# snakers4/silero-vad

Measured on AMD Instinct MI355X. Metric: audio-chunks/sec (32 ms @ 16 kHz), higher is better.
Workload: dtype f32; 1 GPU; configs[1]: synthetic 16 kHz PCM resident in HBM, 512-sample chunks, 4096 streams/GPU x 256 chunks/stream per step, zero initial state; streams_per_gpu=4096

## Files before the change

### silero_vad_amd/csrc/fft_wave.hpp

```cpp
#pragma once
#include <hip/hip_runtime.h>

#include "device_api.hpp"
#include "layout.hpp"

#ifndef VAD_NT_PCM
#define VAD_NT_PCM 0
#endif

namespace vad {
namespace {

using f32x4 = float __attribute__((ext_vector_type(4)));
using u32x4 = unsigned __attribute__((ext_vector_type(4)));

#ifndef VAD_TRACE
#define VAD_TRACE 0
#endif
#ifndef VAD_ABLATE
#define VAD_ABLATE 0
#endif

__device__ constexpr float kCos32[16] = {1.0f, 0.98078525f, 0.9238795f, 0.8314696f, 0.70710677f,
    0.55557024f, 0.38268343f, 0.19509032f, 0.0f, -0.19509032f, -0.38268343f, -0.55557024f,
    -0.70710677f, -0.8314696f, -0.9238795f, -0.98078525f};
__device__ constexpr float kSin32[16] = {0.0f, 0.19509032f, 0.38268343f, 0.55557024f, 0.70710677f,
    0.8314696f, 0.9238795f, 0.98078525f, 1.0f, 0.98078525f, 0.9238795f, 0.8314696f, 0.70710677f,
    0.55557024f, 0.38268343f, 0.19509032f};

constexpr int bitrev(int x, int bits) {
    int r = 0;
    for (int i = 0; i < bits; ++i) r |= ((x >> i) & 1) << (bits - 1 - i);
    return r;
}
constexpr int ilog2(int x) { return x <= 1 ? 0 : 1 + ilog2(x / 2); }

struct Lane {
    int lane, g, j, wave;
    long t;
    long tl;
    long st;
    int b;
    bool tile_valid;
    bool from_tail;
    float sgnA, sgnB;
#if VAD_TRACE
    mutable unsigned long long ts[20] = {};
#endif
};
#if VAD_TRACE
#define VAD_WAVE_STAMP(ln, slot) do { (ln).ts[(slot)] = __builtin_readcyclecounter(); } while (0)
#else
#define VAD_WAVE_STAMP(ln, slot) do { } while (0)
#endif

__device__ __forceinline__ void cvt8(const u32x4 v, float *o) {
#pragma unroll
    for (int k = 0; k < 4; ++k) {
        const int lo = (int)(v[k] << 16) >> 16, hi = (int)v[k] >> 16;
        o[2 * k] = (float)lo * (1.0f / 32768.0f);
        o[2 * k + 1] = (float)hi * (1.0f / 32768.0f);
    }
}
template <int SL, int DEC>
__device__ __forceinline__ void load_vec(const float *p, float (&s)[SL]) {
    if (DEC == 1) {
#pragma unroll
        for (int k = 0; k < SL / 4; ++k) {
            const f32x4 v = VAD_NT_PCM ? __builtin_nontemporal_load(reinterpret_cast<const f32x4 *>(p) + k)
                                       : reinterpret_cast<const f32x4 *>(p)[k];
#pragma unroll
            for (int e = 0; e < 4; ++e) s[4 * k + e] = v[e];
        }
    } else {
#pragma unroll
        for (int i = 0; i < SL; ++i) s[i] = p[i * DEC];
        __builtin_amdgcn_sched_barrier(0);
    }
}
template <int SL, int DEC>
__device__ __forceinline__ void load_vec(const int16_t *p, float (&s)[SL]) {
    if (DEC == 1) {
#pragma unroll
        for (int k = 0; k < SL / 8; ++k)
            cvt8(VAD_NT_PCM ? __builtin_nontemporal_load(reinterpret_cast<const u32x4 *>(p) + k)
                            : reinterpret_cast<const u32x4 *>(p)[k], &s[8 * k]);
    } else {
#pragma unroll
        for (int h = 0; h < 2; ++h) {
#pragma unroll
            for (int i = h * SL / 2; i < (h + 1) * SL / 2; ++i) s[i] = (float)p[i * DEC] * (1.0f / 32768.0f);
            __builtin_amdgcn_sched_barrier(0);
        }
    }
}

template <int Q, typename PcmT, int DEC>
__device__ __forceinline__ void load_slice(float (&s)[2 * Q], const FrontArgs &a, const Lane &ln, const int V) {
    constexpr int SL = 2 * Q, N = 16 * Q;
    const PcmT *row = reinterpret_cast<const PcmT *>(a.pcm) + (size_t)ln.b * a.ld;
    const int sigma = 2 * V + ln.g;
    const int sg = (V == 3 && sigma > 8) ? 8 : sigma;
    const long p0 = (long)SL * (8 * ln.t - 1 + sg);
    const PcmT *src = row + p0 * DEC;
    const PcmT *esrc = row + ((long)N * ln.t + N - SL - 1) * DEC;
    if (ln.from_tail) {
        const PcmT *trow = reinterpret_cast<const PcmT *>(a.tail) + (size_t)ln.b * N * DEC;
        if (sg > 0) src = trow + SL * (sg - 1) * DEC;
        esrc = trow + (N - SL - 1) * DEC;
    }
    if (VAD_ABLATE & 16) {
        const PcmT *r0 = reinterpret_cast<const PcmT *>(a.pcm) + (size_t)(ln.st * 16) * a.ld + (long)SL * 8 * ln.t;
#pragma unroll
        for (int k = 0; k < SL / 4; ++k) {
            const f32x4 v = *reinterpret_cast<const f32x4 *>(reinterpret_cast<const float *>(r0) + (size_t)(k & 15) * a.ld + ln.lane * 4);
#pragma unroll
            for (int e = 0; e < 4; ++e) s[4 * k + e] = v[e];
        }
    } else if (VAD_ABLATE & 32) {
        const float *rr = reinterpret_cast<const float *>(row) + (long)SL * 8 * ln.t;
#pragma unroll
        for (int k = 0; k < SL / 4; ++k) {
            const f32x4 v = *reinterpret_cast<const f32x4 *>(rr + 16 * k + 4 * ln.g + 128 * V);
#pragma unroll
            for (int e = 0; e < 4; ++e) s[4 * k + e] = v[e];
        }
    } else if (DEC == 1) {
        if (V == 0 && ln.t == 0 && ln.g == 0) load_vec<SL, 1>(a.ctx_in + (size_t)ln.b * SL, s);
        else load_vec<SL, 1>(src, s);
    } else if (V == 0) {
        const bool from_ctx = ln.t == 0 && ln.g == 0;
        const PcmT *safe = ln.from_tail ? reinterpret_cast<const PcmT *>(a.tail) + (size_t)ln.b * N * DEC : row;
        load_vec<SL, DEC>(from_ctx ? safe : src, s);
        const f32x4 *c4 = reinterpret_cast<const f32x4 *>(a.ctx_in + (size_t)ln.b * SL);
#pragma unroll
        for (int k = 0; k < SL / 4; ++k) {
            const f32x4 v = c4[k];
#pragma unroll
            for (int e = 0; e < 4; ++e) s[4 * k + e] = from_ctx ? v[e] : s[4 * k + e];
        }
    } else {
        load_vec<SL, DEC>(src, s);
    }
    if (V == 3) {
        if (a.ctx_out && ln.t == a.T - 1 && ln.g == 2 && ln.tile_valid &&
            (ln.st * 16 + ln.j) < a.B) {
            float *o = a.ctx_out + (size_t)ln.b * SL;
#pragma unroll
            for (int k = 0; k < SL / 4; ++k)
                reinterpret_cast<f32x4 *>(o)[k] = f32x4{s[4 * k], s[4 * k + 1], s[4 * k + 2], s[4 * k + 3]};
        }
        const bool rev = ln.g == 3;
        float extra = 0.f;
        if (rev) extra = load_pcm(esrc);
#pragma unroll
        for (int i = 0; i < SL / 2 - 1; ++i) {
            const int k = SL - 2 - i;
            const float lo = s[i], hi = s[k];
            s[i] = rev ? hi : lo;
            s[k] = rev ? lo : hi;
        }
        s[SL - 1] = rev ? extra : s[SL - 1];
    }
}

using f32x2 = float __attribute__((ext_vector_type(2)));

__device__ __forceinline__ f32x2 swap2(f32x2 v) { return f32x2{v.y, v.x}; }
__device__ __forceinline__ f32x2 cmul(f32x2 v, float c, float sn) {
    return __builtin_elementwise_fma(swap2(v), f32x2{-sn, sn}, v * f32x2{c, c});
}

#ifndef VAD_XLANE_SWAP
#define VAD_XLANE_SWAP 1
#endif
__device__ __forceinline__ void trade32(f32x2 &a, f32x2 &b) {
#pragma unroll
    for (int e = 0; e < 2; ++e) {
        const auto r = __builtin_amdgcn_permlane32_swap(__float_as_uint(a[e]), __float_as_uint(b[e]), false, false);
        a[e] = __uint_as_float(r[0]);
        b[e] = __uint_as_float(r[1]);
    }
}
__device__ __forceinline__ void trade16(f32x2 &a, f32x2 &b) {
#pragma unroll
    for (int e = 0; e < 2; ++e) {
        const auto r = __builtin_amdgcn_permlane16_swap(__float_as_uint(a[e]), __float_as_uint(b[e]), false, false);
        a[e] = __uint_as_float(r[0]);
        b[e] = __uint_as_float(r[1]);
    }
}

template <int Q>
__device__ __forceinline__ void fft_inlane(f32x2 (&z)[Q]) {
#pragma unroll
    for (int n = Q; n >= 2; n >>= 1) {
        const int half = n >> 1;
#pragma unroll
        for (int b0 = 0; b0 < Q; b0 += n) {
#pragma unroll
            for (int jx = 0; jx < half; ++jx) {
                const int i0 = b0 + jx, i1 = i0 + half;
                const f32x2 u = z[i0], v = z[i1];
                z[i0] = u + v;
                const f32x2 d = u - v;
                const int tw = jx * (32 / n);
                if (tw == 0) z[i1] = d;
                else if (tw == 8) z[i1] = swap2(d) * f32x2{1.0f, -1.0f};
                else z[i1] = cmul(d, kCos32[tw], -kSin32[tw]);
            }
        }
    }
}

template <int Q>
__device__ __forceinline__ void fft_math(float (&X)[Q + 1], const float (&s)[2 * Q], const float *tab_lds, const Lane &ln);

template <int Q, typename PcmT, int DEC = 1>
__device__ __forceinline__ void fft_frame(float (&X)[Q + 1], const int V, const FrontArgs &a, const float *tab_lds,
                                          const Lane &ln) {
    constexpr int SL = 2 * Q;
    __builtin_amdgcn_sched_barrier(0);
    VAD_WAVE_STAMP(ln, 16 + V);
    float s[SL];
    if (VAD_ABLATE & 4) {
#pragma unroll
        for (int i = 0; i < SL; ++i) s[i] = (float)(ln.lane + i) * 1e-3f;
    } else {
        load_slice<Q, PcmT, DEC>(s, a, ln, V);
    }
#if VAD_TRACE
    asm volatile("s_waitcnt vmcnt(0)" ::: "memory");
    VAD_WAVE_STAMP(ln, 2 + 2 * V);
#endif
    if (VAD_ABLATE & 2) {
#pragma unroll
        for (int k = 0; k < Q; ++k) X[k] = s[k] + s[k + Q];
        X[Q] = s[0];
        return;
    }
    fft_math<Q>(X, s, tab_lds, ln);
    VAD_WAVE_STAMP(ln, 3 + 2 * V);
}

template <int Q>
__device__ __forceinline__ void fft_math(float (&X)[Q + 1], const float (&s)[2 * Q], const float *tab_lds, const Lane &ln) {
    constexpr int SL = 2 * Q;
    constexpr vadl::Tab tb = vadl::make_tab(8 * Q, Q);

    f32x2 z[Q];
    {
        const f32x4 *w = reinterpret_cast<const f32x4 *>(tab_lds + tb.window + SL * ln.g);
#pragma unroll
        for (int k = 0; k < SL / 4; ++k) {
            const f32x4 wv = w[k];
            z[2 * k] = f32x2{s[4 * k], s[4 * k + 1]} * f32x2{wv[0], wv[1]};
            z[2 * k + 1] = f32x2{s[4 * k + 2], s[4 * k + 3]} * f32x2{wv[2], wv[3]};
        }
    }
    const f32x4 *tw1 = reinterpret_cast<const f32x4 *>(tab_lds + tb.tw1 + ln.g * Q * 4);
#if VAD_XLANE_SWAP
    constexpr int H = Q / 2;
    const f32x2 rotA = (ln.g & 1) ? f32x2{0.f, 0.f} : f32x2{1.f, 1.f};
    const f32x2 rotB = (ln.g & 1) ? f32x2{1.f, -1.f} : f32x2{0.f, 0.f};
#pragma unroll
    for (int q = 0; q < H; ++q) trade32(z[q], z[q + H]);
#pragma unroll
    for (int q = 0; q < H; ++q) {
        const f32x2 u = z[q], v = z[q + H], d = u - v;
        z[q] = u + v;
        z[q + H] = __builtin_elementwise_fma(swap2(d), rotB, d * rotA);
    }
#pragma unroll
    for (int q = 0; q < H; ++q) trade32(z[q], z[q + H]);
#pragma unroll
    for (int q = 0; q < H; ++q) trade16(z[q], z[q + H]);
#pragma unroll
    for (int q = 0; q < H; ++q) {
        const f32x2 u = z[q], v = z[q + H];
        z[q] = u + v;
        z[q + H] = u - v;
    }
#pragma unroll
    for (int q = 0; q < H; ++q) trade16(z[q], z[q + H]);
#pragma unroll
    for (int q = 0; q < Q; ++q) {
        const f32x2 x = z[q];
        const f32x4 t = tw1[q];
        z[q] = __builtin_elementwise_fma(swap2(x), f32x2{t[0], t[1]}, x * f32x2{t[2], t[2]});
    }
#else
    const f32x2 sA{ln.sgnA, ln.sgnA}, sB{ln.sgnB, ln.sgnB};
    const f32x2 rotA = ln.g == 3 ? f32x2{0.f, 0.f} : f32x2{1.f, 1.f};
    const f32x2 rotB = ln.g == 3 ? f32x2{1.f, -1.f} : f32x2{0.f, 0.f};
#pragma unroll
    for (int q = 0; q < Q; ++q) {
        f32x2 x = z[q];
        const f32x2 p{__shfl_xor(x.x, 32), __shfl_xor(x.y, 32)};
        x = __builtin_elementwise_fma(sA, x, p);
        x = __builtin_elementwise_fma(swap2(x), rotB, x * rotA);
        const f32x2 r{__shfl_xor(x.x, 16), __shfl_xor(x.y, 16)};
        x = __builtin_elementwise_fma(sB, x, r);
        const f32x4 t = tw1[q];
        z[q] = __builtin_elementwise_fma(swap2(x), f32x2{t[0], t[1]}, x * f32x2{t[2], t[2]});
    }
#endif
    fft_inlane<Q>(z);
    constexpr int LG = ilog2(Q);
    const f32x4 *tw2 = reinterpret_cast<const f32x4 *>(tab_lds + tb.tw2 + ln.g * Q * 4);
    const int src_lane4 = (ln.g >= 2 ? (ln.lane ^ 16) : ln.lane) * 4;
#pragma unroll
    for (int k = 0; k < Q; ++k) {
        const f32x2 u = z[bitrev(k, LG)];
        const int ks = bitrev((Q - k) % Q, LG), kr = bitrev(Q - 1 - k, LG);
        const f32x2 own = z[kr], alt = z[ks];
        const float xr = __int_as_float(__builtin_amdgcn_ds_bpermute(src_lane4, __float_as_int(own.x)));
        const float xi = __int_as_float(__builtin_amdgcn_ds_bpermute(src_lane4, __float_as_int(own.y)));
        const f32x2 p{ln.g == 0 ? alt.x : xr, ln.g == 0 ? alt.y : xi};
        const f32x2 av = __builtin_elementwise_fma(p, f32x2{1.0f, -1.0f}, u);
        const f32x2 ev = __builtin_elementwise_fma(p, f32x2{-1.0f, 1.0f}, u);
        const f32x4 t = tw2[k];
        const f32x2 y = __builtin_elementwise_fma(swap2(ev), f32x2{t[0], t[1]},
                                                  __builtin_elementwise_fma(ev, f32x2{t[2], t[2]}, av));
        const f32x2 yy = y * y;
        X[k] = 0.5f * __builtin_amdgcn_sqrtf(yy.x + yy.y);
    }
    X[Q] = ln.g == 0 ? fabsf(z[0].x - z[0].y) : 0.f;
}

template <int Q>
__device__ __forceinline__ void poison_acc(float &p0, float &p1, const float (&X)[Q + 1]) {
#pragma unroll
    for (int k = 0; k < Q; k += 2) {
        p0 = fmaf(X[k], 0.f, p0);
        p1 = fmaf(X[k + 1], 0.f, p1);
    }
}
__device__ __forceinline__ float poison_nyq(float p0, float p1, float xn0, float xn1, float xn2, float xn3) {
    p0 = fmaf(xn0, 0.f, p0);
    p1 = fmaf(xn1, 0.f, p1);
    p0 = fmaf(xn2, 0.f, p0);
    p1 = fmaf(xn3, 0.f, p1);
    return p0 + p1;
}
__device__ __forceinline__ void poison_into(f32x4 &v, float p) {
    v[0] = __uint_as_float(__float_as_uint(v[0]) | __float_as_uint(p));
}

template <int Q, int V, typename PcmT, int DEC = 1>
__device__ __forceinline__ void fft_pass(float (&X)[Q + 1], const FrontArgs &a, const float *tab_lds, const Lane &ln) {
    fft_frame<Q, PcmT, DEC>(X, V, a, tab_lds, ln);
}

}
}
```

### silero_vad_amd/csrc/kernel_front_f43.hip

```cpp
#include <hip/hip_runtime.h>

#include <type_traits>

#include "fft_wave.hpp"
#include "exact_front.hpp"
#include "front_common.hpp"

namespace vad {
namespace {

#ifndef VAD_BV_BATCH
#define VAD_BV_BATCH 1
#endif
constexpr int kUnitBytes = (int)vadl::kWUnitFloats * 4;
struct Ring {
    unsigned a_cur, a_nxt, a_far;
    unsigned d_cur, d_nxt, d_far;
    const float *src;
    unsigned voff;
    f32x4 c0, c1;
};

__device__ __forceinline__ void ring_request(Ring &r) {
    if (VAD_ABLATE & 8) return;
    unsigned keep_m0;
    asm volatile("s_mov_b32 %0, m0\n\ts_mov_b32 m0, %3\n\ts_nop 0\n\t"
                 "global_load_lds_dwordx4 %1, %2\n\tglobal_load_lds_dwordx4 %1, %2 offset:1024\n\t"
                 "global_load_lds_dwordx4 %1, %2 offset:2048\n\tglobal_load_lds_dwordx4 %1, %2 offset:3072\n\t"
                 "s_mov_b32 m0, %0"
                 : "=&s"(keep_m0) : "v"(r.voff), "s"(r.src), "s"(r.d_far) : "memory");
    r.src += vadl::kWUnitFloats;
}
__device__ __forceinline__ void ring_rotate(Ring &r) {
    const unsigned a = r.a_cur, d = r.d_cur;
    r.a_cur = r.a_nxt; r.a_nxt = r.a_far; r.a_far = a;
    r.d_cur = r.d_nxt; r.d_nxt = r.d_far; r.d_far = d;
}

template <int M, int KG, int AFTER, class BF>
__device__ __forceinline__ void gemm_r(f32x4 (&acc)[M], BF bfun, Ring &r) {
    constexpr int NSTEPS = KG * (M / 2), NU = NSTEPS / 8;
    static_assert(NSTEPS % 8 == 0 && M % 2 == 0, "segments are whole units");
    static_for<0, NU>([&](auto uc) VAD_INLINE {
        constexpr int u = decltype(uc)::value, after = (NU - 1 - u) + AFTER;
        static_for<0, 8>([&](auto sc_) VAD_INLINE {
            constexpr int st = decltype(sc_)::value;
            if constexpr (st == 4 && after >= 1) {
                asm volatile("s_waitcnt vmcnt(0)" ::: "memory");
                if (!(VAD_ABLATE & 1)) __builtin_amdgcn_s_barrier();
                asm volatile("" ::: "memory");
                if constexpr (after >= 2) ring_request(r);
            }
            f32x4 n0 = r.c0, n1 = r.c1;
            if constexpr (st + 1 < 8) {
                n0 = lds4(r.a_cur + (2 * (st + 1)) * 1024);
                n1 = lds4(r.a_cur + (2 * (st + 1) + 1) * 1024);
            } else if constexpr (after >= 1) {
                n0 = lds4(r.a_nxt);
                n1 = lds4(r.a_nxt + 1024);
            }
            __builtin_amdgcn_sched_barrier(0);
            constexpr int i = u * 8 + st, kg = i / (M / 2), mp = 2 * (i % (M / 2));
#if VAD_BV_BATCH
            float bv[4];
#pragma unroll
            for (int ks = 0; ks < 4; ++ks) bv[ks] = bfun(kg * 4 + ks);
            __builtin_amdgcn_sched_barrier(0);
#pragma unroll
            for (int ks = 0; ks < 4; ++ks) {
                acc[mp + 0] = __builtin_amdgcn_mfma_f32_16x16x4f32(r.c0[ks], bv[ks], acc[mp + 0], 0, 0, 0);
                acc[mp + 1] = __builtin_amdgcn_mfma_f32_16x16x4f32(r.c1[ks], bv[ks], acc[mp + 1], 0, 0, 0);
            }
#else
#pragma unroll
            for (int ks = 0; ks < 4; ++ks) {
                const float bv = bfun(kg * 4 + ks);
                acc[mp + 0] = __builtin_amdgcn_mfma_f32_16x16x4f32(r.c0[ks], bv, acc[mp + 0], 0, 0, 0);
                acc[mp + 1] = __builtin_amdgcn_mfma_f32_16x16x4f32(r.c1[ks], bv, acc[mp + 1], 0, 0, 0);
            }
#endif
            __builtin_amdgcn_sched_barrier(0);
            r.c0 = n0;
            r.c1 = n1;
        });
        ring_rotate(r);
    });
}

#ifndef VAD_F43_GEMM_PRIO
#define VAD_F43_GEMM_PRIO 0
#endif
#ifndef VAD_F43_FFT_PRIO
#define VAD_F43_FFT_PRIO 0
#endif
template <int Q, typename PcmT, int DEC>
__global__ void __launch_bounds__(256, 2) front_f43_kernel(const FrontArgs a) {
    using namespace vadl;
    constexpr Tab tb = make_tab(8 * Q, Q);
    constexpr int TABF = (tb.total + 3) / 4 * 4;
    constexpr int RB = w_rb(Q), P = w_parts(Q), KG0 = Q / 4;
    constexpr int PB = Q == 32 ? 2 : 1;
    static_assert(w4_tail0(Q) + 20 == w4_units(Q) && P % PB == 0, "program mismatch");
    __shared__ __attribute__((aligned(16))) float lds[TABF + 3 * (kUnitBytes / 4)];
    float *tab = lds;

    Lane ln;
    ln.lane = threadIdx.x & 63;
    ln.wave = __builtin_amdgcn_readfirstlane(threadIdx.x >> 6);
    ln.g = ln.lane >> 4;
    ln.j = ln.lane & 15;
    const long nst = (a.B + 15) / 16, total = nst * a.nt;
    long wt = (long)blockIdx.x * 4 + ln.wave;
    ln.tile_valid = wt < total;
    if (!ln.tile_valid) wt = total - 1;
    ln.tl = wt % a.nt;
    ln.st = wt / a.nt;
    ln.t = a.t0 + ln.tl;
    const long bb = ln.st * 16 + ln.j;
    ln.b = (int)(bb < a.B ? bb : a.B - 1);
    ln.from_tail = a.tail != nullptr && ln.t == a.T - 1;
    ln.sgnA = ln.g < 2 ? 1.f : -1.f;
    ln.sgnB = (ln.g & 1) ? -1.f : 1.f;
#if VAD_TRACE
    VAD_WAVE_STAMP(ln, 0);
#endif

    Ring ring;
    {
        const unsigned slot0 = (unsigned)(size_t)((__attribute__((address_space(3))) float *)(lds + TABF));
        ring.voff = ln.lane * 16;
        ring.a_cur = slot0 + ring.voff;
        ring.a_nxt = ring.a_cur + kUnitBytes;
        ring.a_far = ring.a_cur + 2 * kUnitBytes;
        ring.d_far = slot0 + (unsigned)ln.wave * 4096u;
        ring.d_cur = ring.d_far + kUnitBytes;
        ring.d_nxt = ring.d_far + 2 * kUnitBytes;
        ring.src = a.wfront + ln.wave * 1024;
        ring_request(ring);
        {   const unsigned d = ring.d_far; ring.d_far = ring.d_cur; ring.d_cur = ring.d_nxt; ring.d_nxt = d; }
        ring_request(ring);
        {   const unsigned d = ring.d_far; ring.d_far = ring.d_cur; ring.d_cur = ring.d_nxt; ring.d_nxt = d; }
    }
    {
        static_assert(tb.total % 4 == 0, "tables are copied as 16-byte vectors");
        constexpr int NV = tb.total / 4, PER = (NV + 255) / 256;
        const f32x4 *src = reinterpret_cast<const f32x4 *>(a.tables);
        f32x4 v[PER];
#pragma unroll
        for (int k = 0; k < PER; ++k) {
            const int i = threadIdx.x + k * 256;
            v[k] = src[i < NV ? i : NV - 1];
        }
#pragma unroll
        for (int k = 0; k < PER; ++k) {
            const int i = threadIdx.x + k * 256;
            if (i < NV) reinterpret_cast<f32x4 *>(tab)[i] = v[k];
        }
    }
    asm volatile("s_waitcnt vmcnt(0)" ::: "memory");
    __syncthreads();
    VAD_WAVE_STAMP(ln, 1);

    float X0[Q + 1], X1[Q + 1], X2[Q + 1], X3[Q + 1];
#pragma unroll
    for (int k = 0; k <= Q; ++k) X1[k] = X2[k] = X3[k] = 0.f;
#pragma clang loop unroll(disable)
    for (int v = 0; v < 4; ++v) {
        if (v >= 3) {
#pragma unroll
            for (int k = 0; k <= Q; ++k) X0[k] = X1[k];
        }
        if (v >= 2) {
#pragma unroll
            for (int k = 0; k <= Q; ++k) X1[k] = X2[k];
        }
        if (v >= 1) {
#pragma unroll
            for (int k = 0; k <= Q; ++k) X2[k] = X3[k];
        }
        if (VAD_F43_FFT_PRIO) __builtin_amdgcn_s_setprio(VAD_F43_FFT_PRIO);
        fft_frame<Q, PcmT, DEC>(X3, v, a, tab, ln);
        if (VAD_F43_FFT_PRIO) __builtin_amdgcn_s_setprio(0);
    }
    if (VAD_F43_GEMM_PRIO) __builtin_amdgcn_s_setprio(VAD_F43_GEMM_PRIO);
    const float xn0 = __shfl(X0[Q], ln.j), xn1 = __shfl(X1[Q], ln.j), xn2 = __shfl(X2[Q], ln.j), xn3 = __shfl(X3[Q], ln.j);
    if (!VAD_NO_EXACT && a.exact_list != nullptr) {
        const SilentMasks sm = silent_chunks(X0[0], X1[0], X2[0], X3[0]);
        const long left = (long)a.B - ln.st * 16;
        const unsigned take = (sm.edge | (a.gx_silent != nullptr ? sm.silent : 0u)) & (left >= 16 ? 0xffffu : ((1u << left) - 1u));
        if (take != 0 && ln.tile_valid) {
            int base = 0;
            if (ln.lane == 0) base = atomicAdd(a.exact_list, __builtin_popcount(take));
            base = __shfl(base, 0);
            if (ln.g == 0 && ((take >> ln.j) & 1))
                a.exact_list[2 + base + __builtin_popcount(take & ((1u << ln.j) - 1u))] =
                    (int)(wt * 16 + ln.j) | (((sm.silent >> ln.j) & 1) ? kExactSilentBit : 0);
        }
    }

#if VAD_F43_EF
#pragma unroll
    for (int k = 0; k < Q; ++k) {
        X3[k] = X3[k] - X1[k];
        X0[k] = X2[k] - X0[k];
    }
    float poison;
    {   float p0 = 0.f, p1 = 0.f;
        poison_acc<Q>(p0, p1, X3);
        poison_acc<Q>(p0, p1, X0);
        poison = poison_nyq(p0, p1, xn0, xn1, xn2, xn3);
    }
#else
    float poison;
    {   float p0 = 0.f, p1 = 0.f;
        poison_acc<Q>(p0, p1, X0);
        poison_acc<Q>(p0, p1, X1);
        poison_acc<Q>(p0, p1, X2);
        poison_acc<Q>(p0, p1, X3);
        poison = poison_nyq(p0, p1, xn0, xn1, xn2, xn3);
    }
#endif
    ring.c0 = lds4(ring.a_cur);
    ring.c1 = lds4(ring.a_cur + 1024);

    f32x4 Z0[4], Z1[4];
    zero<4>(Z0);
    zero<4>(Z1);
#pragma clang loop unroll(disable)
    for (int it = 0; it < P / PB; ++it) {
        f32x4 Ykeep[RB];
        static_for<0, PB>([&](auto pc) VAD_INLINE {
            constexpr int pb = decltype(pc)::value;
            const int row0 = 16 * RB * (it * PB + pb);
            const float *wn = tab + tb.w_nyq + row0;
            f32x4 Y0[RB], Y1[RB], Y2[RB], Y3[RB];
            zero<RB>(Y0);
            zero<RB>(Y1);
            zero<RB>(Y2);
            zero<RB>(Y3);
#if VAD_F43_EF
            {   const Coef k = opaque_coef<kF4, kFm3>();
                gemm_r<RB, KG0, 2>(Y0, [&](int s) VAD_INLINE {
                    return fmaf(fmaf(X2[s], k.p1, X1[s]), k.b, fmaf(X0[s], k.a, X3[s])); }, ring);
                const Coef k2 = opaque_coef<kFm4, kF3>();
                gemm_r<RB, KG0, 2>(Y1, [&](int s) VAD_INLINE {
                    return fmaf(fmaf(X1[s], k2.m1, X2[s]), k2.b, fmaf(X0[s], k2.a, X3[s])); }, ring);
            }
            {   const Coef k = opaque_coef<kF2, kFm2>();
                gemm_r<RB, KG0, 2>(Y2, [&](int s) VAD_INLINE { return fmaf(X0[s], k.a, X3[s]); }, ring);
                gemm_r<RB, KG0, 2>(Y3, [&](int s) VAD_INLINE { return fmaf(X0[s], k.b, X3[s]); }, ring);
            }
#else
            {   const Coef k = opaque_coef<kFm4, kF4>();
                gemm_r<RB, KG0, 2>(Y0, [&](int s) VAD_INLINE {
                    return fmaf(fmaf(X1[s], k.p1, X0[s]), k.a, fmaf(X3[s], k.p1, X2[s])); }, ring);
                gemm_r<RB, KG0, 2>(Y1, [&](int s) VAD_INLINE {
                    return fmaf(fmaf(X1[s], k.m1, X0[s]), k.b, fmaf(X2[s], k.m1, X3[s])); }, ring);
            }
            {   const Coef k = opaque_coef<kF2, kFm2>();
                gemm_r<RB, KG0, 2>(Y2, [&](int s) VAD_INLINE {
                    return fmaf(fmaf(X0[s], k.m1, X2[s]), k.a, fmaf(X1[s], k.m1, X3[s])); }, ring);
                const Coef k2 = opaque_coef<kF2, kFm2>();
                gemm_r<RB, KG0, 2>(Y3, [&](int s) VAD_INLINE {
                    return fmaf(fmaf(X0[s], k2.m1, X2[s]), k2.b, fmaf(X1[s], k2.m1, X3[s])); }, ring);
            }
#endif
#pragma unroll
            for (int m = 0; m < RB; ++m)
#pragma unroll
                for (int r = 0; r < 4; ++r) {
                    const float sm = Y0[m][r] + Y1[m][r], df = Y0[m][r] - Y1[m][r];
                    const float s2 = Y2[m][r] + Y3[m][r], d2 = Y2[m][r] - Y3[m][r];
                    Y0[m][r] = sm + s2;
                    Y1[m][r] = fmaf(2.f, d2, df);
                    Y2[m][r] = fmaf(4.f, s2, sm);
                    Y3[m][r] = fmaf(8.f, d2, df);
                }
#if VAD_F43_EF
            {   const Coef k = opaque_coef<kFm4, kFm025>();
                gemm_r<RB, KG0, 2>(Y0, [&](int s) VAD_INLINE { return fmaf(X1[s], k.a, X3[s]); }, ring);
                gemm_r<RB, KG0, 2>(Y3, [&](int s) VAD_INLINE { return fmaf(X2[s], k.b, -X0[s]); }, ring);
            }
#else
            {   const Coef k = opaque_coef<kFm5, kFm125>();
                gemm_r<RB, KG0, 2>(Y0, [&](int s) VAD_INLINE { return fmaf(X1[s], k.a, X3[s]); }, ring);
                gemm_r<RB, KG0, 2>(Y3, [&](int s) VAD_INLINE { return fmaf(X2[s], k.b, X0[s]); }, ring);
            }
#endif
            nyq_update<RB>(Y0, xn0, wn + 128, ln);
            nyq_update<RB>(Y0, xn1, wn + 256, ln);
            nyq_update<RB>(Y1, xn0, wn, ln);
            nyq_update<RB>(Y1, xn1, wn + 128, ln);
            nyq_update<RB>(Y1, xn2, wn + 256, ln);
            nyq_update<RB>(Y2, xn1, wn, ln);
            nyq_update<RB>(Y2, xn2, wn + 128, ln);
            nyq_update<RB>(Y2, xn3, wn + 256, ln);
            nyq_update<RB>(Y3, xn2, wn, ln);
            nyq_update<RB>(Y3, xn3, wn + 128, ln);
            add_bias<RB>(Y0, tab + tb.b_e0 + row0, ln);
            add_bias<RB>(Y1, tab + tb.b_e0 + row0, ln);
            add_bias<RB>(Y2, tab + tb.b_e0 + row0, ln);
            add_bias<RB>(Y3, tab + tb.b_e0 + row0, ln);
            relu<RB>(Y0);
            relu<RB>(Y1);
            relu<RB>(Y2);
            relu<RB>(Y3);
            if constexpr (Q == 32) {
                auto two = [](const f32x4 (&A)[RB], const f32x4 (&B)[RB], int s) VAD_INLINE {
                    return s < 8 ? A[s >> 2][s & 3] : B[(s - 8) >> 2][s & 3];
                };
                gemm_r<4, 4, 2>(Z0, [&](int s) VAD_INLINE { return two(Y0, Y1, s); }, ring);
                gemm_r<4, 4, 2>(Z1, [&](int s) VAD_INLINE { return two(Y1, Y2, s); }, ring);
                if constexpr (pb == 0) {
#pragma unroll
                    for (int m = 0; m < RB; ++m) Ykeep[m] = Y3[m];
                } else {
                    gemm_r<4, 4, 2>(Z1, [&](int s) VAD_INLINE { return two(Ykeep, Y3, s); }, ring);
                }
            } else {
                auto one = [](const f32x4 (&A)[RB], int s) VAD_INLINE { return A[s >> 2][s & 3]; };
                gemm_r<4, 4, 2>(Z0, [&](int s) VAD_INLINE { return one(Y0, s); }, ring);
                gemm_r<4, 4, 2>(Z0, [&](int s) VAD_INLINE { return one(Y1, s); }, ring);
                gemm_r<4, 4, 2>(Z1, [&](int s) VAD_INLINE { return one(Y1, s); }, ring);
                gemm_r<4, 4, 2>(Z1, [&](int s) VAD_INLINE { return one(Y2, s); }, ring);
                gemm_r<4, 4, 2>(Z1, [&](int s) VAD_INLINE { return one(Y3, s); }, ring);
            }
        });
    }
    add_bias<4>(Z0, tab + tb.b_e1, ln);
    add_bias<4>(Z1, tab + tb.b_e1, ln);
    relu<4>(Z0);
    relu<4>(Z1);
    VAD_WAVE_STAMP(ln, 10);

    f32x4 Vv[4];
    auto bZ0 = [&](int s) VAD_INLINE { return Z0[s >> 2][s & 3]; };
    auto bZ1 = [&](int s) VAD_INLINE { return Z1[s >> 2][s & 3]; };
    auto bV = [&](int s) VAD_INLINE { return Vv[s >> 2][s & 3]; };
    init_bias<4>(Vv, tab + tb.b_e2, ln);
    gemm_r<4, 4, 2>(Vv, bZ0, ring);
    gemm_r<4, 4, 2>(Vv, bZ1, ring);
    relu<4>(Vv);
    f32x4 Fe[8];
    auto bF = [&](int s) VAD_INLINE { return Fe[s >> 2][s & 3]; };
    init_bias<8>(Fe, tab + tb.b_e3, ln);
    gemm_r<8, 4, 2>(Fe, bV, ring);
    relu<8>(Fe);
    poison_into(Fe[0], poison);
    VAD_WAVE_STAMP(ln, 11);

    float *gxt = a.gx + ((size_t)(ln.st * a.nt + ln.tl) * 32) * 256 + ln.lane * 4;
    const float *bg = tab + tb.b_g;
#pragma clang loop unroll(disable)
    for (int q = 0; q < 3; ++q) {
        f32x4 G[8];
        init_bias<8>(G, bg, ln);
        gemm_r<8, 8, 2>(G, bF, ring);
        if (ln.tile_valid) {
#pragma unroll
            for (int m = 0; m < 8; ++m) *reinterpret_cast<f32x4 *>(gxt + (size_t)m * 256) = G[m];
        }
        gxt += 8 * 256;
        bg += 128;
    }
    {
        f32x4 G[8];
        init_bias<8>(G, bg, ln);
        gemm_r<8, 8, 0>(G, bF, ring);
        if (ln.tile_valid) {
#pragma unroll
            for (int m = 0; m < 8; ++m) *reinterpret_cast<f32x4 *>(gxt + (size_t)m * 256) = G[m];
        }
    }
#if VAD_TRACE
    VAD_WAVE_STAMP(ln, 12);
    if (a.trace && ln.lane == 0) {
        long long *tr = a.trace + ((size_t)blockIdx.x * 4 + ln.wave) * 32;
#pragma unroll
        for (int k = 0; k < 20; ++k) tr[k] = (long long)ln.ts[k];
        tr[13] = __builtin_amdgcn_s_getreg((31 << 11) | 4);
        tr[14] = __builtin_amdgcn_s_getreg((31 << 11) | 20);
        tr[15] = (long long)wall_clock64();
    }
#endif
}

}

template <typename PcmT>
hipError_t launch_front_f43(int sr, const FrontArgs &a, hipStream_t s) {
    if (a.B <= 0 || a.nt <= 0) return hipSuccess;
    const long nst = (a.B + 15) / 16, total = nst * a.nt;
    const unsigned grid = (unsigned)((total + 3) / 4);
    if (a.dec > 1 && (sr != 16000 || a.dec > 3)) return hipErrorInvalidValue;
    if (a.dec == 3) hipLaunchKernelGGL((front_f43_kernel<32, PcmT, 3>), dim3(grid), dim3(256), 0, s, a);
    else if (a.dec == 2) hipLaunchKernelGGL((front_f43_kernel<32, PcmT, 2>), dim3(grid), dim3(256), 0, s, a);
    else if (sr == 16000) hipLaunchKernelGGL((front_f43_kernel<32, PcmT, 1>), dim3(grid), dim3(256), 0, s, a);
    else hipLaunchKernelGGL((front_f43_kernel<16, PcmT, 1>), dim3(grid), dim3(256), 0, s, a);
    return hipGetLastError();
}
template hipError_t launch_front_f43<float>(int, const FrontArgs &, hipStream_t);
template hipError_t launch_front_f43<int16_t>(int, const FrontArgs &, hipStream_t);

}
```

Before: 190.5 million chunks/s.

## Prefetch PCM slices ahead of FFT math to overlap loads with compute

Splits slice loading into a request phase (raw vector loads into registers) and a finish phase (convert, context substitution, reversal). The first slice is issued before the table copy and barrier. When the raw slice is small, the next frame's slice is requested before the current frame's FFT math runs, so global-memory latency is hidden behind compute. This costs extra registers to hold the in-flight raw slice and could lower occupancy.

Measured after the change: 188.2 million chunks/s. 1.2% lower.

```diff
diff --git a/silero_vad_amd/csrc/fft_wave.hpp b/silero_vad_amd/csrc/fft_wave.hpp
--- a/silero_vad_amd/csrc/fft_wave.hpp
+++ b/silero_vad_amd/csrc/fft_wave.hpp
@@ -1,5 +1,7 @@
 #pragma once
 #include <hip/hip_runtime.h>
+
+#include <type_traits>
 
 #include "device_api.hpp"
 #include "layout.hpp"
@@ -95,20 +97,102 @@
     }
 }
 
+template <typename PcmT>
+struct SliceSrc {
+    const PcmT *row;
+    const PcmT *src;
+    const PcmT *esrc;
+    const PcmT *safe;
+};
 template <int Q, typename PcmT, int DEC>
-__device__ __forceinline__ void load_slice(float (&s)[2 * Q], const FrontArgs &a, const Lane &ln, const int V) {
+__device__ __forceinline__ SliceSrc<PcmT> slice_src(const FrontArgs &a, const Lane &ln, const int V) {
     constexpr int SL = 2 * Q, N = 16 * Q;
-    const PcmT *row = reinterpret_cast<const PcmT *>(a.pcm) + (size_t)ln.b * a.ld;
+    SliceSrc<PcmT> p;
+    p.row = reinterpret_cast<const PcmT *>(a.pcm) + (size_t)ln.b * a.ld;
     const int sigma = 2 * V + ln.g;
     const int sg = (V == 3 && sigma > 8) ? 8 : sigma;
     const long p0 = (long)SL * (8 * ln.t - 1 + sg);
-    const PcmT *src = row + p0 * DEC;
-    const PcmT *esrc = row + ((long)N * ln.t + N - SL - 1) * DEC;
+    p.src = p.row + p0 * DEC;
+    p.esrc = p.row + ((long)N * ln.t + N - SL - 1) * DEC;
+    p.safe = p.row;
     if (ln.from_tail) {
         const PcmT *trow = reinterpret_cast<const PcmT *>(a.tail) + (size_t)ln.b * N * DEC;
-        if (sg > 0) src = trow + SL * (sg - 1) * DEC;
-        esrc = trow + (N - SL - 1) * DEC;
-    }
+        if (sg > 0) p.src = trow + SL * (sg - 1) * DEC;
+        p.esrc = trow + (N - SL - 1) * DEC;
+        p.safe = trow;
+    }
+    return p;
+}
+template <int Q>
+__device__ __forceinline__ void slice_tail(float (&s)[2 * Q], const float extra, const FrontArgs &a, const Lane &ln) {
+    constexpr int SL = 2 * Q;
+    if (a.ctx_out && ln.t == a.T - 1 && ln.g == 2 && ln.tile_valid &&
+        (ln.st * 16 + ln.j) < a.B) {
+        float *o = a.ctx_out + (size_t)ln.b * SL;
+#pragma unroll
+        for (int k = 0; k < SL / 4; ++k)
+            reinterpret_cast<f32x4 *>(o)[k] = f32x4{s[4 * k], s[4 * k + 1], s[4 * k + 2], s[4 * k + 3]};
+    }
+    const bool rev = ln.g == 3;
+#pragma unroll
+    for (int i = 0; i < SL / 2 - 1; ++i) {
+        const int k = SL - 2 - i;
+        const float lo = s[i], hi = s[k];
+        s[i] = rev ? hi : lo;
+        s[k] = rev ? lo : hi;
+    }
+    s[SL - 1] = rev ? extra : s[SL - 1];
+}
+
+template <int Q, typename PcmT>
+struct RawSlice {
+    using Vec = std::conditional_t<std::is_same<PcmT, float>::value, f32x4, u32x4>;
+    static constexpr int NV = 2 * Q * (int)sizeof(PcmT) / 16;
+    Vec v[NV];
+    float extra;
+};
+template <int Q, typename PcmT>
+__device__ __forceinline__ void slice_request(RawSlice<Q, PcmT> &r, const FrontArgs &a, const Lane &ln, const int V) {
+    using Raw = RawSlice<Q, PcmT>;
+    using Vec = typename Raw::Vec;
+    constexpr int SL = 2 * Q;
+    const SliceSrc<PcmT> p = slice_src<Q, PcmT, 1>(a, ln, V);
+    const bool from_ctx = V == 0 && ln.t == 0 && ln.g == 0;
+    const Vec *q = reinterpret_cast<const Vec *>(p.src);
+    if (from_ctx) q = std::is_same<PcmT, float>::value ? reinterpret_cast<const Vec *>(a.ctx_in + (size_t)ln.b * SL)
+                                                       : reinterpret_cast<const Vec *>(p.safe);
+#pragma unroll
+    for (int k = 0; k < Raw::NV; ++k) r.v[k] = VAD_NT_PCM ? __builtin_nontemporal_load(q + k) : q[k];
+    r.extra = 0.f;
+    if (V == 3 && ln.g == 3) r.extra = load_pcm(p.esrc);
+}
+template <int Q, typename PcmT>
+__device__ __forceinline__ void slice_finish(float (&s)[2 * Q], const RawSlice<Q, PcmT> &r, const FrontArgs &a, const Lane &ln,
+                                             const int V) {
+    constexpr int SL = 2 * Q;
+    if constexpr (std::is_same<PcmT, float>::value) {
+#pragma unroll
+        for (int k = 0; k < SL / 4; ++k)
+#pragma unroll
+            for (int e = 0; e < 4; ++e) s[4 * k + e] = r.v[k][e];
+    } else {
+#pragma unroll
+        for (int k = 0; k < SL / 8; ++k) cvt8(r.v[k], &s[8 * k]);
+        if (V == 0 && ln.t == 0 && ln.g == 0) load_vec<SL, 1>(a.ctx_in + (size_t)ln.b * SL, s);
+    }
+    if (V == 3) slice_tail<Q>(s, r.extra, a, ln);
+}
+
+template <int Q, typename PcmT, int DEC>
+__device__ __forceinline__ void load_slice(float (&s)[2 * Q], const FrontArgs &a, const Lane &ln, const int V) {
+    constexpr int SL = 2 * Q;
+    if (DEC == 1 && !(VAD_ABLATE & (16 | 32))) {
+        RawSlice<Q, PcmT> r;
+        slice_request<Q, PcmT>(r, a, ln, V);
+        slice_finish<Q, PcmT>(s, r, a, ln, V);
+        return;
+    }
+    const SliceSrc<PcmT> p = slice_src<Q, PcmT, DEC>(a, ln, V);
     if (VAD_ABLATE & 16) {
         const PcmT *r0 = reinterpret_cast<const PcmT *>(a.pcm) + (size_t)(ln.st * 16) * a.ld + (long)SL * 8 * ln.t;
 #pragma unroll
@@ -118,20 +202,16 @@
             for (int e = 0; e < 4; ++e) s[4 * k + e] = v[e];
         }
     } else if (VAD_ABLATE & 32) {
-        const float *rr = reinterpret_cast<const float *>(row) + (long)SL * 8 * ln.t;
+        const float *rr = reinterpret_cast<const float *>(p.row) + (long)SL * 8 * ln.t;
 #pragma unroll
         for (int k = 0; k < SL / 4; ++k) {
             const f32x4 v = *reinterpret_cast<const f32x4 *>(rr + 16 * k + 4 * ln.g + 128 * V);
 #pragma unroll
             for (int e = 0; e < 4; ++e) s[4 * k + e] = v[e];
         }
-    } else if (DEC == 1) {
-        if (V == 0 && ln.t == 0 && ln.g == 0) load_vec<SL, 1>(a.ctx_in + (size_t)ln.b * SL, s);
-        else load_vec<SL, 1>(src, s);
     } else if (V == 0) {
         const bool from_ctx = ln.t == 0 && ln.g == 0;
-        const PcmT *safe = ln.from_tail ? reinterpret_cast<const PcmT *>(a.tail) + (size_t)ln.b * N * DEC : row;
-        load_vec<SL, DEC>(from_ctx ? safe : src, s);
+        load_vec<SL, DEC>(from_ctx ? p.safe : p.src, s);
         const f32x4 *c4 = reinterpret_cast<const f32x4 *>(a.ctx_in + (size_t)ln.b * SL);
 #pragma unroll
         for (int k = 0; k < SL / 4; ++k) {
@@ -140,27 +220,12 @@
             for (int e = 0; e < 4; ++e) s[4 * k + e] = from_ctx ? v[e] : s[4 * k + e];
         }
     } else {
-        load_vec<SL, DEC>(src, s);
+        load_vec<SL, DEC>(p.src, s);
     }
     if (V == 3) {
-        if (a.ctx_out && ln.t == a.T - 1 && ln.g == 2 && ln.tile_valid &&
-            (ln.st * 16 + ln.j) < a.B) {
-            float *o = a.ctx_out + (size_t)ln.b * SL;
-#pragma unroll
-            for (int k = 0; k < SL / 4; ++k)
-                reinterpret_cast<f32x4 *>(o)[k] = f32x4{s[4 * k], s[4 * k + 1], s[4 * k + 2], s[4 * k + 3]};
-        }
-        const bool rev = ln.g == 3;
         float extra = 0.f;
-        if (rev) extra = load_pcm(esrc);
-#pragma unroll
-        for (int i = 0; i < SL / 2 - 1; ++i) {
-            const int k = SL - 2 - i;
-            const float lo = s[i], hi = s[k];
-            s[i] = rev ? hi : lo;
-            s[k] = rev ? lo : hi;
-        }
-        s[SL - 1] = rev ? extra : s[SL - 1];
+        if (ln.g == 3) extra = load_pcm(p.esrc);
+        slice_tail<Q>(s, extra, a, ln);
     }
 }
 
diff --git a/silero_vad_amd/csrc/kernel_front_f43.hip b/silero_vad_amd/csrc/kernel_front_f43.hip
--- a/silero_vad_amd/csrc/kernel_front_f43.hip
+++ b/silero_vad_amd/csrc/kernel_front_f43.hip
@@ -141,6 +141,13 @@
         ring_request(ring);
         {   const unsigned d = ring.d_far; ring.d_far = ring.d_cur; ring.d_cur = ring.d_nxt; ring.d_nxt = d; }
     }
+    constexpr bool PIPE = DEC == 1 && !(VAD_ABLATE & (2 | 4 | 16 | 32));
+    constexpr bool ROLL = PIPE && RawSlice<Q, PcmT>::NV <= 8;
+    RawSlice<Q, PcmT> raw;
+    if constexpr (PIPE) {
+        slice_request<Q, PcmT>(raw, a, ln, 0);
+        __builtin_amdgcn_sched_barrier(0);
+    }
     {
         static_assert(tb.total % 4 == 0, "tables are copied as 16-byte vectors");
         constexpr int NV = tb.total / 4, PER = (NV + 255) / 256;
@@ -164,8 +171,21 @@
     float X0[Q + 1], X1[Q + 1], X2[Q + 1], X3[Q + 1];
 #pragma unroll
     for (int k = 0; k <= Q; ++k) X1[k] = X2[k] = X3[k] = 0.f;
+    constexpr int V0 = PIPE && !ROLL ? 1 : 0;
+    if constexpr (V0 == 1) {
+        if (VAD_F43_FFT_PRIO) __builtin_amdgcn_s_setprio(VAD_F43_FFT_PRIO);
+        __builtin_amdgcn_sched_barrier(0);
+        VAD_WAVE_STAMP(ln, 16);
+        VAD_WAVE_STAMP(ln, 2);
+        float s[2 * Q];
+        slice_finish<Q, PcmT>(s, raw, a, ln, 0);
+        fft_math<Q>(X3, s, tab, ln);
+        VAD_WAVE_STAMP(ln, 3);
+        __builtin_amdgcn_sched_barrier(0);
+        if (VAD_F43_FFT_PRIO) __builtin_amdgcn_s_setprio(0);
+    }
 #pragma clang loop unroll(disable)
-    for (int v = 0; v < 4; ++v) {
+    for (int v = V0; v < 4; ++v) {
         if (v >= 3) {
 #pragma unroll
             for (int k = 0; k <= Q; ++k) X0[k] = X1[k];
@@ -179,7 +199,23 @@
             for (int k = 0; k <= Q; ++k) X2[k] = X3[k];
         }
         if (VAD_F43_FFT_PRIO) __builtin_amdgcn_s_setprio(VAD_F43_FFT_PRIO);
-        fft_frame<Q, PcmT, DEC>(X3, v, a, tab, ln);
+        if constexpr (PIPE) {
+            __builtin_amdgcn_sched_barrier(0);
+            VAD_WAVE_STAMP(ln, 16 + v);
+            if (!ROLL) slice_request<Q, PcmT>(raw, a, ln, v);
+#if VAD_TRACE
+            asm volatile("s_waitcnt vmcnt(0)" ::: "memory");
+            VAD_WAVE_STAMP(ln, 2 + 2 * v);
+#endif
+            float s[2 * Q];
+            slice_finish<Q, PcmT>(s, raw, a, ln, v);
+            if (ROLL && v < 3) slice_request<Q, PcmT>(raw, a, ln, v + 1);
+            __builtin_amdgcn_sched_barrier(0);
+            fft_math<Q>(X3, s, tab, ln);
+            VAD_WAVE_STAMP(ln, 3 + 2 * v);
+        } else {
+            fft_frame<Q, PcmT, DEC>(X3, v, a, tab, ln);
+        }
         if (VAD_F43_FFT_PRIO) __builtin_amdgcn_s_setprio(0);
     }
     if (VAD_F43_GEMM_PRIO) __builtin_amdgcn_s_setprio(VAD_F43_GEMM_PRIO);
```
